# yu45020/Text_Segmentation_Image_Inpainting

Hardware: NVIDIA H100
Metric: PartialConv UNet 512x512 images/sec (fwd+bwd) (higher is better)
Workload: dtype bf16

## Files before the change

### text_segmentation_image_inpainting_b200/csrc/conv_tc.cu

```cuda
#include <cuda.h>
#include <stdlib.h>
#include <string.h>

#include <algorithm>

#include "pcb_common.cuh"
#include "pcb_ptx.cuh"
#include "pcb_tc_epi.cuh"

namespace {

__device__ __forceinline__ float warp_transpose_sum(float (&v)[32], int lane) {
#pragma unroll
    for (int off = 16, n = 32; off >= 1; off >>= 1, n >>= 1) {
        const bool upper = (lane & off) != 0;
#pragma unroll
        for (int i = 0; i < 16; ++i) {
            if (i < (n >> 1)) {
                const float send = upper ? v[i] : v[i + (n >> 1)];
                const float keep = upper ? v[i + (n >> 1)] : v[i];
                v[i] = keep + __shfl_xor_sync(0xffffffffu, send, off);
            }
        }
    }
// ... 621 lines not shown
                            const uint8_t *mk = P.parts[p].mask + static_cast<long long>(img) * (P.h >> mup) * (P.w >> mup);
                            for (int tr = 0; tr < P.kh; ++tr) {
                                const int y = oy - P.pad_h + tr * P.dil;
                                if (y < 0 || y >= P.h) continue;
#pragma unroll
                                for (int r = 0; r < FR; ++r) {
                                    const int row = t + TMA_FIX_THREADS * r, x = ox - P.pad_w + row;
                                    if (row < BLOCK_M + hx && x >= 0 && x < P.w && __ldg(mk + (y >> mup) * (P.w >> mup) + (x >> mup)) == 0)
                                        b[r] |= 1u << (p * 8 + tr);
                                }
                            }
                        }
                    };
                    uint32_t nb_bits[FR];
                    load_bits(tile0, nb_bits);
                    for (int tile = tile0; tile < num_tiles && !dead; tile += tstep) {
                        uint32_t cb_bits[FR];
#pragma unroll
                        for (int r = 0; r < FR; ++r) cb_bits[r] = nb_bits[r];
                        load_bits(tile + tstep, nb_bits);
                        if (MODE == 1 && !tile_active((tile % n_tiles) * BLOCK_N)) continue;
                        for (int tr = 0; tr < P.kh && !dead; ++tr) {
#pragma unroll
                            for (int p = 0; p < TC_MAX_PARTS; ++p) {
                                if (p >= np) break;
                                bool hole[FR], mine = false;
#pragma unroll
                                for (int r = 0; r < FR; ++r) { hole[r] = (cb_bits[r] >> (p * 8 + tr)) & 1u; mine = mine || hole[r]; }
                                const bool any_hole = __any_sync(0xffffffffu, mine);
                                const int nb = ((MODE == 0) ? P.parts[p].kext : P.dc_kext) / BLOCK_K;
                                for (int cb = 0; cb < nb; ++cb) {
                                    if (!ptx::mbar_wait(bar_full + 8 * s, ph, P.abort_flag, 122)) { dead = true; break; }
                                    if (any_hole) {
#pragma unroll
                                        for (int r = 0; r < FR; ++r)
                                            if (hole[r]) zero_row(t + TMA_FIX_THREADS * r);
                                        ptx::fence_proxy_async_smem();
                                    }
                                    __syncwarp();
                                    if (lane == 0) ptx::mbar_arrive(bar_fixed + 8 * s);
                                    if (++s == S) { s = 0; ph ^= 1; }
                                }
                                if (dead) break;
                            }
                        }
                    }
                }
            }
        }
    }

}


constexpr int SP_MAX_ITEMS = 40;
struct SpItem { int dx, dy, wk; };
struct SpTable {
    int n_items;
    SpItem it[SP_MAX_ITEMS];
};

template <int BLOCK_N>
__global__ void __maxnreg__(TMA_REGS)
pconv_tc_sp_kernel(const __grid_constant__ TcParams P, const __grid_constant__ SpTable TB, const __grid_constant__ CUtensorMap tmap_w,
                   const __grid_constant__ CUtensorMap tmap_a) {
    constexpr uint32_t B_BYTES = BLOCK_N * 128;
    constexpr uint32_t STAGE = A_STAGE_BYTES + B_BYTES;
    extern __shared__ uint8_t smem_raw[];
    const uint32_t smem_base = align1024(ptx::smem_u32(smem_raw));
    const int S = P.stages;
    const uint32_t sBar = smem_base + S * STAGE;
    const uint32_t bar_full = sBar, bar_empty = sBar + 16 * MAX_RING;
    const uint32_t acc_full = sBar + 24 * MAX_RING, acc_empty = acc_full + 8;
    const uint32_t s_acc = sBar + TMA_BAR_BYTES + EPI_STAT_SMEM_BYTES;
    bf16 *acc_stage = reinterpret_cast<bf16 *>(smem_raw + (s_acc - ptx::smem_u32(smem_raw)));

    const int warp = __shfl_sync(0xffffffffu, threadIdx.x >> 5, 0), lane = threadIdx.x & 31;
    const int n_tiles = P.ncols / BLOCK_N;
    const int m_tiles = (P.m_total + BLOCK_M - 1) / BLOCK_M;
    const int num_tiles = m_tiles * n_tiles;
    const int tile0 = static_cast<int>(blockIdx.x), tstep = static_cast<int>(gridDim.x);
    const int plane = P.w * P.h;
    const int nbk = P.dc_kext / BLOCK_K;
    const int klast = min(4, (P.dc_c8 - (nbk - 1) * BLOCK_K + 15) >> 4);

    if (threadIdx.x == 0) {
        for (int s = 0; s < MAX_RING; ++s) { ptx::mbar_init(bar_full + 8 * s, 1); ptx::mbar_init(bar_empty + 8 * s, 2); }
        ptx::mbar_init(acc_full, MMA_WARPS); ptx::mbar_init(acc_empty, EPI_WARPS);
        ptx::fence_mbar_init();
    }
    if (warp == 8 && lane == 0) { ptx::prefetch_tmap(&tmap_w); ptx::prefetch_tmap(&tmap_a); }
    __syncthreads();

    if (warp < MMA_WARPS) {
        ptx::setmaxnreg_inc<TMA_CONSUMER_REGS>();
        const int e = warp, g = warp >> 2;
        const bool leader = (threadIdx.x & 127) == 0;
        const uint64_t desc_a0 = ptx::make_smem_desc(smem_base + g * 64 * 128, 16, 1024);
        const uint64_t desc_b0 = ptx::make_smem_desc(smem_base + A_STAGE_BYTES, 16, 1024);
        const uint32_t stage16 = STAGE >> 4;
        int s = 0;
        uint32_t ph = 0, aph = 1;
        bool dead = false;
        for (int tile = tile0; tile < num_tiles && !dead; tile += tstep) {
            float acc[BLOCK_N / 2];
            zero_acc(acc);
// ... 824 lines not shown
bool even_upsampled_parts(const pcb_conv *c) {
    for (int p = 0; p < c->nparts; ++p)
        if (c->parts[p].x_up && ((c->h | c->w) & 1)) return false;
    return true;
}

bool tma_fwd_ok(const pcb_conv *c, int *bw, int *bh, int *bn) {
    if (is_rowpack(c) || !tile_box(c->wo, c->ho, bw, bh, bn)) return false;
    if (c->stride > 2 || *bw * c->stride > 256 || *bh * c->stride > 256) return false;
    return even_upsampled_parts(c);
}

bool tma_dgrad_s2_ok(const pcb_conv *c, int *bw, int *bh, int *bn) {
    if (c->stride != 2 || c->dil != 1 || c->kh < 2 || c->kw < 2 || ((c->h | c->w) & 1) || c->ho != c->h / 2 || c->wo != c->w / 2) return false;
    return tile_box(c->w / 2, c->h / 2, bw, bh, bn);
}

int class_kw(const pcb_conv *c, int px) { return (c->kw - ((px + c->pad_w) & 1) + 1) / 2; }

bool tma_wgrad_ok(const pcb_conv *c, int *bw, int *bh, int *bn) {
    return !is_rowpack(c) && c->stride <= 2 && kblock_box(c->wo, c->ho, bw, bh, bn) && even_upsampled_parts(c);
}

size_t up_bytes(const pcb_conv *c, int p) {
    return (static_cast<size_t>(c->n) * c->h * c->w * rup(c->parts[p].c, 8) * 2 + 255) / 256 * 256;
}
size_t tapmask_bytes(const pcb_conv *c) {
    return (static_cast<size_t>(c->nparts) * c->n * c->ho * c->wo * sizeof(uint64_t) + 255) / 256 * 256;
}

size_t tma_fixed_smem(int block_n) {
    return 1024 + TMA_BAR_BYTES + EPI_STAT_SMEM_BYTES + bf16_stage_bytes(block_n);
}

template <int BLOCK_N, int MODE, bool HALO>
int launch_tma_n(TcParams &P, const CUtensorMap &tw, const CUtensorMap &ta0, const CUtensorMap &ta1, cudaStream_t st) {
    const int nb = HALO ? P.kw : 1;
    const size_t a_room = (static_cast<size_t>(BLOCK_M + (HALO ? (P.kw - 1) * P.dil : 0)) * 128 + 1023) / 1024 * 1024;
    const size_t stage = a_room + static_cast<size_t>(nb) * BLOCK_N * 128;
    const size_t fixed = tma_fixed_smem(BLOCK_N);
    P.stages = static_cast<int>(std::min<size_t>(MAX_RING, (MAX_SMEM - fixed) / stage));
    PCB_CHECK(P.stages >= 2, "TMA-fed conv: stage of %zu bytes does not fit twice", stage);
    const size_t smem = fixed + P.stages * stage;
    auto kern = pconv_tc_tma_kernel<BLOCK_N, MODE, HALO>;
    PCB_SMEM_OPT_IN(kern, MAX_SMEM);
    const int m_tiles = (P.m_total + BLOCK_M - 1) / BLOCK_M;
    const int num_tiles = m_tiles * (P.ncols / BLOCK_N);
    const int grid = std::min(num_tiles, pcb_num_sms());
    kern<<<grid, TMA_THREADS, smem, st>>>(P, tw, ta0, ta1);
    PCB_LAUNCH_CHECK();
    return 0;
}

template <int MODE>
int launch_tma(TcParams &P, const CUtensorMap &tw, const CUtensorMap &ta0, const CUtensorMap &ta1, int bn, bool halo, cudaStream_t st) {
    PCB_CHECK(!(halo && bn == 256), "TMA-fed conv: no 256-wide row-halo tiles");
    if (halo) {
        if (bn == 128) return launch_tma_n<128, MODE, true>(P, tw, ta0, ta1, st);
        if (bn == 64) return launch_tma_n<64, MODE, true>(P, tw, ta0, ta1, st);
        return launch_tma_n<32, MODE, true>(P, tw, ta0, ta1, st);
    }
    if (bn == 256) return launch_tma_n<256, MODE, false>(P, tw, ta0, ta1, st);
    if (bn == 128) return launch_tma_n<128, MODE, false>(P, tw, ta0, ta1, st);
    if (bn == 64) return launch_tma_n<64, MODE, false>(P, tw, ta0, ta1, st);
    return launch_tma_n<32, MODE, false>(P, tw, ta0, ta1, st);
}

bool halo_stages_fit(int kw, int dil, int block_n) {
    const size_t stage = (static_cast<size_t>(128 + (kw - 1) * dil) * 128 + 1023) / 1024 * 1024 + static_cast<size_t>(kw) * block_n * 128;
    return 3 * stage + acc_stage_bytes(block_n) <= RING_BUDGET;
}

bool halo_ok(int kw, int dil, int bw, int bh, int bn, int block_n) {
    return bw == 128 && bh == 1 && bn == 1 && kw >= 2 && 128 + (kw - 1) * dil <= 256 && halo_stages_fit(kw, dil, block_n);
}

int pick_bn(int cols, long long m_total, bool fwd, int sms) {
    const long long m_tiles = (m_total + BLOCK_M - 1) / BLOCK_M;
    if (cols <= 32) return 32;
    auto waves = [&](int b) { return (m_tiles * (cols / b) + sms - 1) / sms; };
    if (cols % 256 == 0 && 2 * waves(256) <= waves(128) && (!fwd || waves(256) == 1)) return 256;
    int bn = (cols % 128 == 0) ? 128 : 64;
    while (bn > 32 && cols % (bn / 2) == 0 && m_tiles * (cols / bn) < sms / 2) bn /= 2;
    return bn;
}

template <int MODE>
int launch_tc(TcParams &P, const CUtensorMap &tm, int bn, cudaStream_t st) {
    return (bn == 128) ? launch_persistent<128, MODE>(P, tm, st) : launch_persistent<64, MODE>(P, tm, st);
}

struct ClassStreams { cudaStream_t aux[3]; cudaEvent_t ev_fork, ev_join[3]; bool ready; };
int class_streams(ClassStreams **out) {
    static thread_local ClassStreams cs_all[PCB_MAX_DEVICES] = {};
    ClassStreams &CS = cs_all[pcb_cur_device()];
    if (!CS.ready) {
        for (int i = 0; i < 3; ++i) {
            PCB_CUDA(cudaStreamCreateWithFlags(&CS.aux[i], cudaStreamNonBlocking));
            PCB_CUDA(cudaEventCreateWithFlags(&CS.ev_join[i], cudaEventDisableTiming));
        }
        PCB_CUDA(cudaEventCreateWithFlags(&CS.ev_fork, cudaEventDisableTiming));
        CS.ready = true;
    }
    *out = &CS;
    return 0;
}

struct SpAxis { int e0[2], ne[2], tapbits[2][4]; bool ok; };

// ... 108 lines not shown
    const int num_tiles = ((P.m_total + BLOCK_M - 1) / BLOCK_M) * (P.ncols / BLOCK_N);
    const int grid = std::min(num_tiles, pcb_num_sms());
    kern<<<grid, TMA_THREADS, smem, st>>>(P, TB, tw, ta);
    PCB_LAUNCH_CHECK();
    return 0;
}

int sp_dgrad_up(const pcb_conv *c, const SpPlan &S, const Layout &L, const void *dc, int dc_cstride, const bf16 *w_sp_dg, void *dx_u, int dx_cstride,
                int *flag, cudaStream_t st) {
    const int hs = c->h / 2, ws = c->w / 2;
    const long long m_src = static_cast<long long>(c->n) * hs * ws;
    TcParams P;
    base_params(P, c, L);
    P.h = hs; P.w = ws; P.m_total = static_cast<int>(m_src);
    P.sub = 1; P.py = 0; P.px = 0; P.fh = hs; P.fw = ws;
    P.nparts = 1;
    memset(P.parts, 0, sizeof(P.parts));
    TcPart &pt = P.parts[0];
    pt.c = c->parts[S.pu].c; pt.c8 = S.c8_u; pt.kext = S.kext_u; pt.koff = 0; pt.mask = c->parts[S.pu].mask; pt.mup = 0;
    pt.dx = static_cast<bf16 *>(dx_u); pt.dx_cstride = dx_cstride;
    PCB_CHECK(dx_cstride % 8 == 0 && dx_cstride >= S.c8_u && (reinterpret_cast<uintptr_t>(dx_u) & 15) == 0, "sub-pixel dgrad: dx must be 16-byte aligned with a channel stride that is a multiple of 8");
    P.dc = static_cast<const bf16 *>(dc); P.dc_cstride = dc_cstride; P.dc_c8 = rup(c->cout, 8); P.dc_kext = L.cout64;
    P.abort_flag = flag;
    P.ncols = S.kext_u;
    P.box_w = S.bw; P.box_h = S.bh; P.box_n = S.bn;
    const int bn = S.block_n;
    SpTable TB;
    memset(&TB, 0, sizeof(TB));
    int ni = 0;
    for (int cls = 0; cls < 4; ++cls) {
        const int py = cls >> 1, px = cls & 1;
        const int ney = S.ay.ne[py], nex = S.ax.ne[px];
        for (int e = 0; e < ney; ++e)
            for (int f = 0; f < nex; ++f) {
                SpItem &it = TB.it[ni++];
                it.dx = px - 2 * (S.ax.e0[px] + f); it.dy = py - 2 * (S.ay.e0[py] + e);
                it.wk = (S.eoff[cls] + e * nex + f) * L.cout64;
            }
    }
    TB.n_items = ni;
    CUtensorMap ta, tw;
    if (int rc = make_tmap_nhwc(&ta, dc, P.dc_c8, c->wo, c->ho, c->n, dc_cstride, S.bw, S.bh, S.bn, 2)) return rc;
    if (int rc = make_tmap_2d(&tw, w_sp_dg, rup(S.kext_u, 128), S.kd_sp, S.kd_sp, bn)) return rc;
    return (bn == 64) ? launch_sp_n<64>(P, TB, tw, ta, st) : launch_sp_n<32>(P, TB, tw, ta, st);
}

enum TcRoute { ROUTE_NONE, ROUTE_STEM, ROUTE_K2R, ROUTE_SMALLCO, ROUTE_TMA, ROUTE_TMA_S2, ROUTE_GATHER };

struct DirPlan {
    TcRoute route;
    int box_w, box_h, box_n;
    int bn;
    bool halo;
};

struct TcPlan {
    bool ok;
    Layout L;
    long long m_out, m_in;
    size_t fwd_elems, dg_elems;
    size_t extra_fwd_off, extra_dg_off;
    size_t sp_off;
    size_t workspace;
    size_t up_off[TC_MAX_PARTS];
    DirPlan fwd, dg, wg;
    bool fwd_tapmask, wg_tapmask;
    StemPlan stem;
    K2rPlan k2r;
    SpPlan sp;
    bool cls_halo[4];
    bool cls_fork;
    bool fuses_epilogue;
    bool dg_fuses_relu;
    bool dg_at_source;
};

TcPlan tc_plan(const pcb_conv *c) {
    TcPlan T;
    memset(&T, 0, sizeof(T));
    T.sp.pu = T.sp.ps = -1;
    if (!common_ok(c)) return T;
    T.ok = true;
    const int sms = pcb_num_sms();
    T.L = layout_of(c);
    const Layout &L = T.L;
    T.m_out = static_cast<long long>(c->n) * c->ho * c->wo;
    T.m_in = static_cast<long long>(c->n) * c->h * c->w;
    bool any_mask = false;
    for (int p = 0; p < c->nparts; ++p) any_mask = any_mask || (c->parts[p].mask != nullptr);
    const bool smallco = !L.rowpack && pcb_smallco_eligible(c);
    if (L.rowpack) T.stem = pcb_stem_plan(c);
    if (smallco) T.k2r = pcb_k2r_plan(c);
    const bool stem = T.stem.ok, k2r = T.k2r.ok;
    if (!L.rowpack && !smallco) T.sp = sp_plan(c, L, sms);

    T.fwd_elems = static_cast<size_t>(L.rows_f) * L.kf;
    T.sp_off = static_cast<size_t>(rup(L.ktap, 128)) * L.kd;
    T.dg_elems = L.rowpack ? 0 : T.sp_off;
    if (T.sp.ok) T.dg_elems += static_cast<size_t>(T.sp.sp_dg_elems);
    T.extra_fwd_off = (T.fwd_elems + 63) / 64 * 64;
    T.extra_dg_off = (T.sp_off + 63) / 64 * 64;
    if (k2r) {
        T.fwd_elems = T.extra_fwd_off + T.k2r.fwd_extra;
        T.dg_elems = T.extra_dg_off + T.k2r.dg_extra;
    }
    if (stem) T.fwd_elems = T.extra_fwd_off + T.stem.fwd_extra;

    int bw, bh, bn;
    const bool fwd_tma = tma_fwd_ok(c, &bw, &bh, &bn);
    DirPlan &F = T.fwd;
    if (stem) F.route = ROUTE_STEM;
    else if (k2r) F.route = ROUTE_K2R;
    else if (smallco) F.route = ROUTE_SMALLCO;
    else if (fwd_tma) {
        F.route = ROUTE_TMA;
        F.box_w = bw; F.box_h = bh; F.box_n = bn;
        F.bn = pick_bn(c->cout <= 32 ? 32 : L.rows_f, T.m_out, true, sms);
        F.halo = c->stride == 1 && c->kh <= 8 && halo_ok(c->kw, c->dil, bw, bh, bn, F.bn);
        T.fwd_tapmask = any_mask && !F.halo;
    } else {
        F.route = ROUTE_GATHER;
        F.bn = L.bn_f;
        T.fwd_tapmask = true;
    }

    DirPlan &D = T.dg;
    if (k2r) D.route = ROUTE_K2R;
    else if (smallco) D.route = ROUTE_SMALLCO;
    else if (L.rowpack) D.route = ROUTE_NONE;
    else if (c->stride == 1 && tile_box(c->w, c->h, &bw, &bh, &bn)) {
        D.route = ROUTE_TMA;
        D.box_w = bw; D.box_h = bh; D.box_n = bn;
        D.bn = pick_bn(L.ktap, T.m_in, false, sms);
        D.halo = c->kh <= 8 && halo_ok(c->kw, c->dil, bw, bh, bn, D.bn);
    } else if (tma_dgrad_s2_ok(c, &bw, &bh, &bn)) {
        D.route = ROUTE_TMA_S2;
        D.box_w = bw; D.box_h = bh; D.box_n = bn;
        const long long m_class = static_cast<long long>(c->n) * (c->h / 2) * (c->w / 2);
        D.bn = pick_bn(L.ktap, m_class, false, sms);
        for (int cls = 0; cls < 4; ++cls) T.cls_halo[cls] = halo_ok(class_kw(c, cls & 1), 1, bw, bh, bn, D.bn);
        T.cls_fork = ((m_class + BLOCK_M - 1) / BLOCK_M) * (L.ktap / D.bn) < sms;
    } else {
        D.route = ROUTE_GATHER;
        D.bn = (L.ktap % 128 == 0) ? 128 : 64;
    }

    const bool wg_tma = tma_wgrad_ok(c, &bw, &bh, &bn);
    DirPlan &W = T.wg;
    if (stem) W.route = ROUTE_STEM;
    else if (k2r) W.route = ROUTE_K2R;
    else if (smallco) W.route = ROUTE_SMALLCO;
    else if (wg_tma) {
        W.route = ROUTE_TMA;
        W.box_w = bw; W.box_h = bh; W.box_n = bn;
        W.halo = c->stride == 1 && c->kw == 3 && bw == 64 && bh == 1 && bn == 1 && 64 + (c->kw - 1) * c->dil <= 256;
        W.bn = (c->cout > 64 && T.m_out >= 128 * 64) ? 128 : 64;
        T.wg_tapmask = any_mask;
    } else {
        W.route = ROUTE_GATHER;
        T.wg_tapmask = true;
    }

    if (k2r) T.workspace = T.k2r.workspace;
    else if (stem) T.workspace = std::max(T.stem.workspace, tapmask_bytes(c));
    else {
        T.workspace = tapmask_bytes(c);
        if (fwd_tma || wg_tma)
            for (int p = 0; p < c->nparts; ++p)
                if (c->parts[p].x_up) { T.up_off[p] = T.workspace; T.workspace += up_bytes(c, p); }
    }

    T.fuses_epilogue = !smallco;
    T.dg_fuses_relu = c->nparts == 1 && !T.sp.ok && D.route == ROUTE_TMA;
    T.dg_at_source = smallco ? k2r : T.sp.ok;
    return T;
}

int a_operand_maps(const pcb_conv *c, const TcPlan &T, void *workspace, int bx, int by, int bn, CUtensorMap (&ta)[TC_MAX_PARTS],
                   int *use_fix, cudaStream_t st) {
    memset(ta, 0, sizeof(ta));
    for (int p = 0; p < c->nparts; ++p) {
        const pcb_part &pt = c->parts[p];
        const void *src = pt.x;
        long long cs = pt.x_cstride;
        const int c8 = rup(pt.c, 8);
        if (pt.x_up) {
            bf16 *up = reinterpret_cast<bf16 *>(static_cast<uint8_t *>(workspace) + T.up_off[p]);
// ... 65 lines not shown
    if (T.fwd.route == ROUTE_STEM) return pcb_stem_weight_prepare(c, T.stem, w_master, wf + T.extra_fwd_off, zero_padding, st);
    if (T.fwd.route == ROUTE_K2R) {
        PCB_CHECK(w_dgrad != nullptr, "kernel-to-row weights need the dgrad operand buffer");
        return pcb_k2r_weight_prepare(c, T.k2r, w_master, wf + T.extra_fwd_off, wd + T.extra_dg_off, zero_padding, st);
    }
    if (T.sp.ok) {
        PCB_CHECK(w_dgrad != nullptr, "sub-pixel weights need the dgrad operand buffer");
        return sp_weight_prepare(c, T.sp, L, w_master, wd + T.sp_off, st);
    }
    return 0;
}

int pcb_tc_forward_mask_pass(const pcb_conv *c, uint64_t *tapmask, cudaStream_t st) {
    const TcPlan T = tc_plan(c);
    PCB_CHECK(T.m_out < (1ll << 31), "problem too large");
    return T.fwd_tapmask ? launch_tapmask(c, tapmask, st) : 0;
}

bool pcb_tc_fuses_epilogue(const pcb_conv *c) { return tc_plan(c).fuses_epilogue; }

int pcb_tc_forward_ws(const pcb_conv *c, const void *w_fwd, const float *bias, void *y, int y_cstride, const float *msum,
                      uint64_t *tapmask, bool mask_pass_done, double *bn_sums, const pcb_ep *ep, cudaStream_t st) {
    int *flag = abort_flag_ptr();
    PCB_CHECK(flag != nullptr, "cudaMalloc(abort flag) failed");
    const TcPlan T = tc_plan(c);
    const Layout &L = T.L;
    const DirPlan &F = T.fwd;
    PCB_CHECK(T.m_out < (1ll << 31), "problem too large");
    PCB_CHECK(y_cstride % 8 == 0 && y_cstride >= c->cout, "tensor-core forward: y channel stride must be a multiple of 8 and >= cout");
    PCB_CHECK(bn_sums == nullptr || T.fuses_epilogue, "fused BatchNorm statistics requested from a kernel that does not produce them");
    PCB_CHECK(ep == nullptr || T.fuses_epilogue, "fused BatchNorm + activation requested from a kernel that does not apply it");
    if (!mask_pass_done && T.fwd_tapmask)
        if (int rc = launch_tapmask(c, tapmask, st)) return rc;
    const bf16 *wf = static_cast<const bf16 *>(w_fwd);
    if (F.route == ROUTE_STEM) return pcb_stem_forward(c, T.stem, wf + T.extra_fwd_off, bias, y, y_cstride, msum, tapmask, bn_sums, ep, st);
    if (F.route == ROUTE_K2R) return pcb_k2r_forward(c, T.k2r, smallco_layout(L), w_fwd, wf + T.extra_fwd_off, bias, y, y_cstride, msum, tapmask, st);
    if (F.route == ROUTE_SMALLCO) return pcb_smallco_forward(c, smallco_layout(L), w_fwd, bias, y, y_cstride, msum, st);
    TcParams P;
    base_params(P, c, L);
    P.m_total = static_cast<int>(T.m_out);
    fill_parts(c, L, P.parts, tapmask, T.m_out);
    P.bias = bias; P.msum = msum; P.y = static_cast<bf16 *>(y); P.y_cstride = y_cstride; P.abort_flag = flag;
    P.bn_sums = bn_sums; P.bn_c = c->cout;
    set_ep(P, ep);
    P.ncols = L.rows_f;
    CUtensorMap tm;
    if (int rc = make_tmap_2d(&tm, w_fwd, L.rows_f, L.kf, L.kf, F.bn)) return rc;
    if (F.route == ROUTE_TMA) {
        P.box_w = F.box_w; P.box_h = F.box_h; P.box_n = F.box_n;
        CUtensorMap ta[TC_MAX_PARTS];
        if (int rc = a_operand_maps(c, T, tapmask, F.box_w + (F.halo ? (c->kw - 1) * c->dil : 0), F.box_h, F.box_n, ta, &P.use_fix, st)) return rc;
        P.ncols = (c->cout <= 32) ? 32 : L.rows_f;
        P.wk_base = 0; P.wk_col = L.ktap; P.wk_row = c->kw * L.ktap;
        return launch_tma<0>(P, tm, ta[0], ta[1], F.bn, F.halo, st);
    }
    return launch_tc<0>(P, tm, F.bn, st);
}

bool pcb_tc_dgrad_fuses_relu(const pcb_conv *c) { return tc_plan(c).dg_fuses_relu; }

int pcb_tc_dgrad(const pcb_conv *c, const void *dc, int dc_cstride, const void *w_dgrad, void *const *dx, const int *dx_cstride,
                 cudaStream_t st, const void *relu_x, int relu_cstride) {
    const TcPlan T = tc_plan(c);
    const Layout &L = T.L;
    const DirPlan &D = T.dg;
    PCB_CHECK(D.route != ROUTE_NONE, "data gradient of a row-packed (cin <= 8) tensor-core layer: set force_generic and pass KRSC weights");
    PCB_CHECK(w_dgrad != nullptr && (reinterpret_cast<uintptr_t>(dc) & 15) == 0, "pcb_pconv_backward_data: w_dgrad required / dc misaligned");
    PCB_CHECK(relu_x == nullptr || (T.dg_fuses_relu && relu_cstride % 8 == 0 && relu_cstride >= rup(c->cin, 8) &&
                                    (reinterpret_cast<uintptr_t>(relu_x) & 15) == 0),
              "tensor-core dgrad: the ReLU backward is fused only on the TMA-fed stride-1 kernel (16-byte aligned input, channel stride %% 8 == 0)");
    int *flag = abort_flag_ptr();
    PCB_CHECK(flag != nullptr, "cudaMalloc(abort flag) failed");
    PCB_CHECK(T.m_in < (1ll << 31), "problem too large");
    PCB_CHECK(dc_cstride % 8 == 0 && dc_cstride >= rup(c->cout, 8), "tensor-core dgrad: dc channel stride must be a multiple of 8");
    const bf16 *wd = static_cast<const bf16 *>(w_dgrad);
    if (D.route == ROUTE_K2R) return pcb_k2r_dgrad(c, T.k2r, smallco_layout(L), dc, dc_cstride, w_dgrad, wd + T.extra_dg_off, dx, dx_cstride, st);
    if (D.route == ROUTE_SMALLCO) return pcb_smallco_dgrad(c, smallco_layout(L), dc, dc_cstride, w_dgrad, dx, dx_cstride, st);
    const SpPlan &SPL = T.sp;
    void *dx_local[TC_MAX_PARTS] = {nullptr, nullptr};
    for (int p = 0; p < c->nparts && p < TC_MAX_PARTS; ++p) dx_local[p] = dx[p];
    if (SPL.ok) {
        if (dx[SPL.pu] != nullptr)
            if (int rc = sp_dgrad_up(c, SPL, L, dc, dc_cstride, wd + T.sp_off, dx[SPL.pu], dx_cstride[SPL.pu], flag, st)) return rc;
        dx_local[SPL.pu] = nullptr;
        if (SPL.ps < 0 || dx[SPL.ps] == nullptr) return 0;
    }
    dx = dx_local;
    TcParams P;
    base_params(P, c, L);
    P.m_total = static_cast<int>(T.m_in);
    fill_parts(c, L, P.parts, nullptr, 0);
    for (int p = 0; p < c->nparts; ++p) {
        P.parts[p].dx = static_cast<bf16 *>(dx[p]);
        P.parts[p].dx_cstride = dx_cstride[p];
        PCB_CHECK(!dx[p] || (dx_cstride[p] % 8 == 0 && dx_cstride[p] >= P.parts[p].c8 && (reinterpret_cast<uintptr_t>(dx[p]) & 15) == 0),
                  "tensor-core dgrad: dx[%d] must be 16-byte aligned with a channel stride that is a multiple of 8", p);
    }
    P.dc = static_cast<const bf16 *>(dc); P.dc_cstride = dc_cstride; P.dc_c8 = rup(c->cout, 8); P.dc_kext = L.cout64;
    P.relu_x = static_cast<const bf16 *>(relu_x); P.relu_cstride = relu_cstride;
    P.abort_flag = flag;
    P.ncols = L.ktap;
    CUtensorMap tm;
    if (int rc = make_tmap_2d(&tm, w_dgrad, rup(L.ktap, 128), L.kd, L.kd, D.bn)) return rc;
    if (D.route == ROUTE_TMA) {
        P.box_w = D.box_w; P.box_h = D.box_h; P.box_n = D.box_n;
        P.wk_base = 0; P.wk_col = L.cout64; P.wk_row = c->kw * L.cout64;
        CUtensorMap ta;
        if (int rc = make_tmap_nhwc(&ta, dc, P.dc_c8, c->wo, c->ho, c->n, dc_cstride, D.box_w + (D.halo ? (c->kw - 1) * c->dil : 0), D.box_h, D.box_n, 1)) return rc;
        return launch_tma<1>(P, tm, ta, ta, D.bn, D.halo, st);
    }
    if (D.route == ROUTE_TMA_S2) {
        const int hh = c->h / 2, hw = c->w / 2;
        P.box_w = D.box_w; P.box_h = D.box_h; P.box_n = D.box_n;
        const bool fork = T.cls_fork;
        ClassStreams *CS = nullptr;
        if (fork) {
            if (int rc = class_streams(&CS)) return rc;
            PCB_CUDA(cudaEventRecord(CS->ev_fork, st));
        }
        for (int cls = 0; cls < 4; ++cls) {
            TcParams Q = P;
            const int py = cls >> 1, px = cls & 1;
            const int tr0 = (py + c->pad_h) & 1, tc0 = (px + c->pad_w) & 1;
            Q.kh = (c->kh - tr0 + 1) / 2; Q.kw = class_kw(c, px);
            Q.pad_h = (py + c->pad_h - tr0) / 2; Q.pad_w = (px + c->pad_w - tc0) / 2;
            Q.h = hh; Q.w = hw; Q.stride = 1; Q.dil = 1;
            Q.m_total = static_cast<int>(static_cast<long long>(c->n) * hh * hw);
            Q.sub = 2; Q.py = py; Q.px = px; Q.fh = c->h; Q.fw = c->w;
            Q.wk_base = (tr0 * c->kw + tc0) * L.cout64; Q.wk_row = 2 * c->kw * L.cout64; Q.wk_col = 2 * L.cout64;
            const bool halo = T.cls_halo[cls];
            CUtensorMap ta;
            if (int rc = make_tmap_nhwc(&ta, dc, P.dc_c8, c->wo, c->ho, c->n, dc_cstride, Q.box_w + (halo ? Q.kw - 1 : 0), Q.box_h, Q.box_n, 1)) return rc;
            cudaStream_t cs = (fork && cls > 0) ? CS->aux[cls - 1] : st;
            if (fork && cls > 0) PCB_CUDA(cudaStreamWaitEvent(cs, CS->ev_fork, 0));
            if (int rc = launch_tma<1>(Q, tm, ta, ta, D.bn, halo, cs)) return rc;
            if (fork && cls > 0) {
                PCB_CUDA(cudaEventRecord(CS->ev_join[cls - 1], cs));
                PCB_CUDA(cudaStreamWaitEvent(st, CS->ev_join[cls - 1], 0));
            }
        }
        return 0;
    }
    return launch_tc<1>(P, tm, D.bn, st);
}


template <int BLOCK_N, int T, bool HALO>
int launch_wgrad_tma(WgParams &P, const CUtensorMap &tdc, const CUtensorMap &ta0, const CUtensorMap &ta1, cudaStream_t st) {
    const int rows_a = 64 + (HALO ? (P.kw - 1) * P.dil : 0);
    PCB_CHECK(rows_a <= (HALO ? 3 : 1) * WGRAD_FIX_THREADS, "TMA-fed wgrad: %d-row A blocks exceed the fixer warps", rows_a);
    const size_t a_blk = (static_cast<size_t>(rows_a) * 128 + 1023) / 1024 * 1024;
    const size_t stage = (HALO ? 1 : T) * 2 * a_blk + static_cast<size_t>(BLOCK_N) * 128;
    P.stages = static_cast<int>(std::min<size_t>(MAX_RING, RING_BUDGET / stage));
    PCB_CHECK(P.stages >= 2, "TMA-fed wgrad: stage of %zu bytes does not fit twice", stage);
    const size_t smem = 1024 + P.stages * stage + 24 * MAX_RING;
    auto kern = pconv_tc_wgrad_tma_kernel<BLOCK_N, T, HALO>;
    PCB_SMEM_OPT_IN(kern, MAX_SMEM);
    P.tap_groups = HALO ? P.kh : (P.kh * P.kw + T - 1) / T;
    P.ci_tiles = (P.ktap + 127) / 128;
    const int co_tiles = (P.cout + BLOCK_N - 1) / BLOCK_N;
    const int base_ctas = co_tiles * P.tap_groups * P.ci_tiles;
    const int total_kb = (P.m_total + 63) / 64;
// ... 78 lines not shown
```

### text_segmentation_image_inpainting_b200/csrc/pcb_tc_epi.cuh

```cuda
#pragma once
#include <cuda.h>

#include "pcb_common.cuh"
#include "pcb_ptx.cuh"

namespace {

constexpr int BLOCK_M = 128;
constexpr int BLOCK_K = 64;
constexpr int A_STAGE_BYTES = BLOCK_M * 128;
constexpr int NUM_PRODUCER_THREADS = 128;
constexpr int TC_MAX_PARTS = 2;
constexpr int MMA_WARPS = 8;
constexpr int MMA_THREADS = MMA_WARPS * 32;
constexpr int acc_pitch(int block_n) { return block_n + 4; }
constexpr int acc_stage_bytes(int block_n) { return BLOCK_M * acc_pitch(block_n) * 4; }

inline int rup(int v, int m) { return (v + m - 1) / m * m; }

struct TcPart {
    const bf16 *x;
    const uint64_t *tapmask;
    const uint8_t *mask;
    bf16 *dx;
// ... 173 lines not shown
                ob[j] = __floats2bfloat162_rn(f.x * scale, f.y * scale);
            }
        }
        if (MODE == 1 && P.relu_x != nullptr && nstore > 0) {
            const uint4 *xr = reinterpret_cast<const uint4 *>(P.relu_x + er.mo * P.relu_cstride + xlocal);
#pragma unroll 1
            for (int j = 0; j < 4; ++j) {
                if (j * 8 >= nstore) break;
                const uint4 xv = xr[j];
                const __nv_bfloat162 *xb = reinterpret_cast<const __nv_bfloat162 *>(&xv);
                __nv_bfloat162 *ob = reinterpret_cast<__nv_bfloat162 *>(&o[j]);
#pragma unroll
                for (int k = 0; k < 4; ++k) {
                    const float2 xf = __bfloat1622float2(xb[k]);
                    const __nv_bfloat162 z = __float2bfloat162_rn(0.f);
                    ob[k] = __halves2bfloat162(xf.x <= 0.f ? z.x : ob[k].x, xf.y <= 0.f ? z.y : ob[k].y);
                }
            }
        }
        if (nstore > 0) {
            uint4 *dst = reinterpret_cast<uint4 *>(orow);
#pragma unroll
            for (int j = 0; j < 4; ++j)
                if (j * 8 < nstore) dst[j] = o[j];
        }
        if (stats) {
            const float live = er.rvalid ? 1.f : 0.f;
            const __nv_bfloat162 *ob = reinterpret_cast<const __nv_bfloat162 *>(srow + c0);
            float cs = 0.f, cq = 0.f;
#pragma unroll 1
            for (int h = 0; h < 2; ++h) {
                float v[16];
#pragma unroll
                for (int j = 0; j < 8; ++j) {
                    const float2 f = __bfloat1622float2(ob[8 * h + j]);
                    v[2 * j] = f.x * live; v[2 * j + 1] = f.y * live;
                }
                const float s = warp_transpose_sum16(v, lane);
#pragma unroll
                for (int j = 0; j < 8; ++j) {
                    const float2 f = __bfloat1622float2(ob[8 * h + j]);
                    const float a = f.x * live, b = f.y * live;
                    v[2 * j] = a * a; v[2 * j + 1] = b * b;
                }
                const float q = warp_transpose_sum16(v, lane);
                if ((lane >> 4) == h) { cs = s; cq = q; }
            }
            s_stat[c0 + lane] += cs;
            s_stat[EPI_STAT_SQ + c0 + lane] += cq;
        }
    }
}

template <int BLOCK_N, int MODE, typename TileFn>
__device__ __forceinline__ void tma_epilogue_warps(const TcParams &P, int tile0, int tstep, int num_tiles, TileFn tile_origin,
                                                   const bf16 *stage, uint32_t acc_full, uint32_t acc_empty, float *s_stat,
                                                   int &stat_n0, int w, int lane, int code) {
    const int row = w * 32 + lane;
    if (s_stat) {
        for (int i = lane; i < EPI_STAT_SLICE; i += 32) s_stat[i] = 0.f;
        __syncwarp();
    }
    uint32_t ph = 0;
    for (int tile = tile0; tile < num_tiles; tile += tstep) {
        int m0, n0;
        tile_origin(tile, m0, n0);
        if (n0 < 0) continue;
        if (s_stat && n0 != stat_n0) {
            if (stat_n0 >= 0) tc_stats_flush<BLOCK_N>(P, s_stat, lane, stat_n0, 0, BLOCK_N, EPI_STAT_SQ);
            stat_n0 = n0;
        }
        const EpiRow er = tc_epi_row<MODE>(P, m0 + row, false);
        if (!__all_sync(0xffffffffu, ptx::mbar_wait(acc_full, ph, P.abort_flag, code))) { stat_n0 = -1; return; }
        ph ^= 1;
        tc_epilogue_bf16<BLOCK_N, MODE>(P, er, stage + row * bf16_pitch(BLOCK_N), lane, n0, s_stat);
        __syncwarp();
        if (lane == 0) ptx::mbar_arrive(acc_empty);
    }
}

struct ConsRows {
    float inv[2];
    bool hole[2];
};
template <int MODE>
__device__ __forceinline__ ConsRows cons_rows(const TcParams &P, int m0, int e, int lane) {
    ConsRows cr;
#pragma unroll
    for (int h = 0; h < 2; ++h) {
        cr.inv[h] = 0.f; cr.hole[h] = false;
        if (MODE == 0) {
            const EpiRow er = tc_epi_row<0>(P, m0 + 64 * (e >> 2) + 16 * (e & 3) + (lane >> 2) + 8 * h);
            cr.inv[h] = er.inv; cr.hole[h] = er.hole;
        }
    }
    return cr;
}

template <int BLOCK_N, int MODE>
__device__ __forceinline__ void stage_acc_bf16(const TcParams &P, const float (&acc)[BLOCK_N / 2], bf16 *stage, int e, int lane, int n0,
                                               const ConsRows &cr) {
    constexpr int PITCH = bf16_pitch(BLOCK_N);
    const int r0 = 64 * (e >> 2) + 16 * (e & 3) + (lane >> 2), c0 = 2 * (lane & 3);
    const bool has_bias = (MODE == 0) && (P.bias != nullptr);
    const bool ep = (MODE == 0) && (P.ep_on != 0);
    const bool ep_aff = ep && (P.ep_scale != nullptr);
#pragma unroll
    for (int j = 0; j < BLOCK_N / 8; ++j) {
        const int col = n0 + 8 * j + c0;
        float b0 = 0.f, b1 = 0.f, s0 = 1.f, s1 = 1.f, t0 = 0.f, t1 = 0.f;
        if (MODE == 0) {
            const bool in0 = col < P.cout, in1 = col + 1 < P.cout;
            if (has_bias) { if (in0) b0 = __ldg(P.bias + col); if (in1) b1 = __ldg(P.bias + col + 1); }
            if (ep_aff) {
                if (in0) { s0 = __ldg(P.ep_scale + col); t0 = __ldg(P.ep_shift + col); }
                if (in1) { s1 = __ldg(P.ep_scale + col + 1); t1 = __ldg(P.ep_shift + col + 1); }
            }
        }
#pragma unroll
        for (int h = 0; h < 2; ++h) {
            float a = acc[4 * j + 2 * h], b = acc[4 * j + 2 * h + 1];
            if (MODE == 0) {
                a = cr.hole[h] ? 0.f : fmaf(a, cr.inv[h], b0);
                b = cr.hole[h] ? 0.f : fmaf(b, cr.inv[h], b1);
                if (ep) {
                    a = apply_act(fmaf(a, s0, t0), P.ep_act, P.ep_slope);
                    b = apply_act(fmaf(b, s1, t1), P.ep_act, P.ep_slope);
                }
                if (col >= P.cout) a = 0.f;
                if (col + 1 >= P.cout) b = 0.f;
            }
            *reinterpret_cast<__nv_bfloat162 *>(stage + (r0 + 8 * h) * PITCH + 8 * j + c0) = __floats2bfloat162_rn(a, b);
        }
    }
}

template <int BLOCK_N, int MODE>
__device__ __forceinline__ bool tma_stage_tile(const TcParams &P, const float (&acc)[BLOCK_N / 2], bf16 *stage, uint32_t acc_full,
                                               uint32_t acc_empty, uint32_t &ph, int e, int lane, int n0, const ConsRows &cr, int code) {
    if (!__all_sync(0xffffffffu, ptx::mbar_wait(acc_empty, ph, P.abort_flag, code))) return false;
    ph ^= 1;
    stage_acc_bf16<BLOCK_N, MODE>(P, acc, stage, e, lane, n0, cr);
    __syncwarp();
    if (lane == 0) ptx::mbar_arrive(acc_full);
    return true;
}

}
```

Measured before the change: 1163.

## Add pair-tile row-halo TMA conv kernel sharing weight stages across two M sub-tiles

Adds a kernel variant in which each CTA processes two adjacent 128-row row-halo sub-tiles. The two consumer warpgroups share each weight (B) stage, and A and W get separate ring buffers sized independently. The change targets weight-load traffic and barrier overhead per unit of MMA work on large stride-1 forward and dgrad convolutions. It costs more shared memory per stage, more accumulator registers (two sets per warp), and fewer tiles to spread across SMs. The planner enables it only when the tile count is at least twice the SM count.

```diff
diff --git a/text_segmentation_image_inpainting_b200/csrc/conv_tc.cu b/text_segmentation_image_inpainting_b200/csrc/conv_tc.cu
--- a/text_segmentation_image_inpainting_b200/csrc/conv_tc.cu
+++ b/text_segmentation_image_inpainting_b200/csrc/conv_tc.cu
@@ -697,6 +697,279 @@
 
 }
 
+constexpr size_t PAIR_BAR_BYTES = 40 * MAX_RING + 16;
+
+template <int BLOCK_N, int MODE, bool HALO, int PAIRS>
+__global__ void __maxnreg__(TMA_REGS)
+pconv_tc_tma_kernel(const __grid_constant__ TcParams P, const __grid_constant__ CUtensorMap tmap_w,
+                    const __grid_constant__ CUtensorMap tmap_a0, const __grid_constant__ CUtensorMap tmap_a1) {
+    static_assert(HALO && PAIRS == 2 && (BLOCK_N == 64 || BLOCK_N == 128), "pair tiles: two row-halo sub-tiles, N = 64 or 128");
+    constexpr int PM = PAIRS * BLOCK_M;
+    constexpr uint32_t B_BYTES = BLOCK_N * 128;
+    extern __shared__ uint8_t smem_raw[];
+    const uint32_t smem_base = align1024(ptx::smem_u32(smem_raw));
+    const int SA = P.ring_a, SW = P.ring_b;
+    const int hx = (P.kw - 1) * P.dil;
+    const int rows_sub = BLOCK_M + hx;
+    const uint32_t A_BYTES = static_cast<uint32_t>(rows_sub) * 128u;
+    const uint32_t A_ROOM = (A_BYTES + 1023u) & ~1023u;
+    const uint32_t ASTAGE = PAIRS * A_ROOM;
+    const uint32_t sW = smem_base + SA * ASTAGE;
+    const uint32_t sBar = sW + SW * B_BYTES;
+    const uint32_t a_full = sBar, a_fixed = sBar + 8 * MAX_RING, a_empty = sBar + 16 * MAX_RING;
+    const uint32_t w_full = sBar + 24 * MAX_RING, w_empty = sBar + 32 * MAX_RING;
+    const uint32_t acc_full = sBar + 40 * MAX_RING, acc_empty = acc_full + 8;
+    const uint32_t s_stat_addr = sBar + PAIR_BAR_BYTES;
+    const uint32_t s_acc = s_stat_addr + EPI_STAT_SMEM_BYTES;
+    uint8_t *smem_gen = smem_raw + (smem_base - ptx::smem_u32(smem_raw));
+
+    const int warp = __shfl_sync(0xffffffffu, threadIdx.x >> 5, 0), lane = threadIdx.x & 31;
+    const int np = (MODE == 0) ? P.nparts : 1;
+    const int n_tiles = P.ncols / BLOCK_N;
+    const int num_tiles = (P.m_total / PM) * n_tiles;
+    const int tile0 = static_cast<int>(blockIdx.x), tstep = static_cast<int>(gridDim.x);
+    const bool fix = (MODE == 0) && P.use_fix;
+
+    auto tile_active = [&](int n0) -> bool {
+        if (MODE == 0) return true;
+        for (int p = 0; p < P.nparts; ++p)
+            if (P.parts[p].dx && n0 < P.parts[p].koff + P.parts[p].kext && n0 + BLOCK_N > P.parts[p].koff) return true;
+        return false;
+    };
+
+    if (threadIdx.x == 0) {
+        for (int s = 0; s < MAX_RING; ++s) {
+            ptx::mbar_init(a_full + 8 * s, 1); ptx::mbar_init(a_fixed + 8 * s, TMA_FIX_THREADS / 32); ptx::mbar_init(a_empty + 8 * s, 2);
+            ptx::mbar_init(w_full + 8 * s, 1); ptx::mbar_init(w_empty + 8 * s, 2);
+        }
+        ptx::mbar_init(acc_full, MMA_WARPS); ptx::mbar_init(acc_empty, EPI_WARPS);
+        ptx::fence_mbar_init();
+    }
+    if (warp == 8 && lane == 0) { ptx::prefetch_tmap(&tmap_w); ptx::prefetch_tmap(&tmap_a0); if (np > 1) ptx::prefetch_tmap(&tmap_a1); }
+    __syncthreads();
+
+    bf16 *acc_stage = reinterpret_cast<bf16 *>(smem_gen + (s_acc - smem_base));
+    if (warp < MMA_WARPS) {
+        ptx::setmaxnreg_inc<TMA_CONSUMER_REGS>();
+        const int g = warp >> 2, we = warp & 3;
+        const bool leader = (threadIdx.x & 127) == 0;
+        const uint32_t ready = fix ? a_fixed : a_full;
+        const uint64_t desc_a0 = ptx::make_smem_desc(smem_base + g * A_ROOM, 16, 1024);
+        const uint64_t desc_b0 = ptx::make_smem_desc(sW, 16, 1024);
+        const uint32_t astage16 = ASTAGE >> 4, b16 = B_BYTES >> 4, half16 = (64 * 128) >> 4;
+        const int shift0 = (MODE == 1) ? hx * 8 : 0;
+        const int dshift = (MODE == 1) ? -P.dil * 8 : P.dil * 8;
+        int nb0, nb1 = 0, kl0, kl1 = 4;
+        {
+            const int kext = (MODE == 0) ? P.parts[0].kext : P.dc_kext, c8 = (MODE == 0) ? P.parts[0].c8 : P.dc_c8;
+            nb0 = kext / BLOCK_K; kl0 = min(4, (c8 - (nb0 - 1) * BLOCK_K + 15) >> 4);
+            if (MODE == 0 && np > 1) { nb1 = P.parts[1].kext / BLOCK_K; kl1 = min(4, (P.parts[1].c8 - (nb1 - 1) * BLOCK_K + 15) >> 4); }
+        }
+        int sa = 0, sw = 0;
+        uint32_t pha = 0, phw = 0, aph = 1;
+        bool dead = false;
+        for (int tile = tile0; tile < num_tiles && !dead; tile += tstep) {
+            const int n0 = (tile % n_tiles) * BLOCK_N;
+            if (!tile_active(n0)) continue;
+            const int m0 = (tile / n_tiles) * PM + g * BLOCK_M;
+            const ConsRows cr0 = cons_rows<MODE>(P, m0, we, lane), cr1 = cons_rows<MODE>(P, m0, we + 4, lane);
+            float acc0[BLOCK_N / 2], acc1[BLOCK_N / 2];
+            zero_acc(acc0);
+            zero_acc(acc1);
+            int held_a = -1, held_w = -1;
+            for (int r = 0; r < P.kh && !dead; ++r) {
+#pragma unroll
+                for (int p = 0; p < TC_MAX_PARTS; ++p) {
+                    const int nbp = (p == 0) ? nb0 : nb1, klast = (p == 0) ? kl0 : kl1;
+                    for (int cb = 0; cb < nbp && !dead; ++cb) {
+                        if (!__all_sync(0xffffffffu, ptx::mbar_wait(ready + 8 * sa, pha, P.abort_flag, 144))) { dead = true; break; }
+                        uint64_t da = desc_a0 + static_cast<uint64_t>(sa * astage16 + shift0);
+                        const int ksteps = (cb + 1 < nbp) ? 4 : klast;
+                        for (int tc = 0; tc < P.kw; ++tc, da += dshift) {
+                            if (!__all_sync(0xffffffffu, ptx::mbar_wait(w_full + 8 * sw, phw, P.abort_flag, 145))) { dead = true; break; }
+                            const uint64_t db = desc_b0 + static_cast<uint64_t>(sw * b16);
+                            ptx::wgmma_fence();
+                            if (ksteps == 4) {
+#pragma unroll
+                                for (int k = 0; k < 4; ++k) {
+                                    ptx::wgmma_bf16<BLOCK_N, 0, 0>(acc0, da + 2 * k, db + 2 * k);
+                                    ptx::wgmma_bf16<BLOCK_N, 0, 0>(acc1, da + half16 + 2 * k, db + 2 * k);
+                                }
+                            } else {
+                                for (int k = 0; k < ksteps; ++k) {
+                                    ptx::wgmma_bf16<BLOCK_N, 0, 0>(acc0, da + 2 * k, db + 2 * k);
+                                    ptx::wgmma_bf16<BLOCK_N, 0, 0>(acc1, da + half16 + 2 * k, db + 2 * k);
+                                }
+                            }
+                            ptx::wgmma_commit();
+                            ptx::wgmma_wait<1>();
+                            if (leader) {
+                                if (held_w >= 0) ptx::mbar_arrive(w_empty + 8 * held_w);
+                                if (held_a >= 0) ptx::mbar_arrive(a_empty + 8 * held_a);
+                            }
+                            held_a = -1;
+                            held_w = sw;
+                            if (++sw == SW) { sw = 0; phw ^= 1; }
+                        }
+                        held_a = sa;
+                        if (++sa == SA) { sa = 0; pha ^= 1; }
+                    }
+                    if (dead) break;
+                }
+            }
+            ptx::wgmma_wait<0>();
+            ptx::wgmma_fence_regs(acc0);
+            ptx::wgmma_fence_regs(acc1);
+            if (leader) {
+                if (held_w >= 0) ptx::mbar_arrive(w_empty + 8 * held_w);
+                if (held_a >= 0) ptx::mbar_arrive(a_empty + 8 * held_a);
+            }
+            if (dead) break;
+            if (!__all_sync(0xffffffffu, ptx::mbar_wait(acc_empty, aph, P.abort_flag, 146))) break;
+            aph ^= 1;
+            stage_acc_bf16_sets<BLOCK_N, MODE, true>(P, acc0, acc1, acc_stage + g * BLOCK_M * bf16_pitch(BLOCK_N), we, lane, n0, cr0, cr1);
+            __syncwarp();
+            if (lane == 0) ptx::mbar_arrive(acc_full);
+        }
+    } else {
+        ptx::setmaxnreg_dec<TMA_SUPPORT_REGS>();
+        if (warp >= EPI_WARP0) {
+            const int w = warp - EPI_WARP0;
+            float *s_stat = (MODE == 0 && P.bn_sums != nullptr)
+                                ? reinterpret_cast<float *>(smem_gen + (s_stat_addr - smem_base)) + w * EPI_STAT_SLICE : nullptr;
+            int stat_n0 = -1;
+            auto origin = [&](int tile, int &m0, int &n0) {
+                m0 = (tile / n_tiles) * PM; n0 = (tile % n_tiles) * BLOCK_N;
+                if (!tile_active(n0)) n0 = -1;
+            };
+            tma_epilogue_warps<BLOCK_N, MODE, PAIRS>(P, tile0, tstep, num_tiles, origin, acc_stage, acc_full, acc_empty, s_stat, stat_n0, w,
+                                                     lane, 147);
+            ptx::named_sync(1, EPI_WARPS * 32);
+            if (s_stat != nullptr && stat_n0 >= 0) tc_stats_final<BLOCK_N>(P, s_stat - w * EPI_STAT_SLICE, w, lane, stat_n0);
+        } else if (warp == 8) {
+            int sa = 0, sw = 0;
+            uint32_t pha = 1, phw = 1;
+            const int plane = (MODE == 0) ? P.ho * P.wo : P.h * P.w;
+            const int pwid = (MODE == 0) ? P.wo : P.w;
+            const int kext0 = (MODE == 0) ? P.parts[0].kext : P.dc_kext, kext1 = (MODE == 0 && np > 1) ? P.parts[1].kext : 0;
+            const int dstep = (MODE == 0) ? P.dil : -P.dil;
+            bool dead = false;
+            for (int tile = tile0; tile < num_tiles && !dead; tile += tstep) {
+                const int mp = (tile / n_tiles) * PM, n0 = (tile % n_tiles) * BLOCK_N;
+                if (!tile_active(n0)) continue;
+                int xs[PAIRS], ys[PAIRS], img[PAIRS];
+#pragma unroll
+                for (int j = 0; j < PAIRS; ++j) {
+                    const int m = mp + j * BLOCK_M;
+                    img[j] = m / plane;
+                    const int rem = m - img[j] * plane, oy = rem / pwid, ox = rem - oy * pwid;
+                    xs[j] = (MODE == 0) ? ox - P.pad_w : ox + P.pad_w - hx;
+                    ys[j] = (MODE == 0) ? oy - P.pad_h : oy + P.pad_h;
+                }
+                int krow = P.wk_base;
+                for (int tr = 0; tr < P.kh && !dead; ++tr, krow += P.wk_row) {
+                    int kidx = krow;
+#pragma unroll
+                    for (int p = 0; p < TC_MAX_PARTS; ++p) {
+                        const int kext = (p == 0) ? kext0 : kext1;
+                        const CUtensorMap *ma = (p == 0) ? &tmap_a0 : &tmap_a1;
+                        for (int c0 = 0; c0 < kext && !dead; c0 += BLOCK_K, kidx += BLOCK_K) {
+                            if (!__all_sync(0xffffffffu, ptx::mbar_wait(a_empty + 8 * sa, pha, P.abort_flag, 141))) { dead = true; break; }
+                            if (ptx::elect_one()) {
+                                const uint32_t full = a_full + 8 * sa, dst = smem_base + sa * ASTAGE;
+                                ptx::mbar_arrive_expect_tx(full, PAIRS * A_BYTES);
+#pragma unroll
+                                for (int j = 0; j < PAIRS; ++j) ptx::tma_load_4d(dst + j * A_ROOM, ma, c0, xs[j], ys[j] + tr * dstep, img[j], full);
+                            }
+                            __syncwarp();
+                            if (++sa == SA) { sa = 0; pha ^= 1; }
+                            for (int tc = 0; tc < P.kw; ++tc) {
+                                if (!__all_sync(0xffffffffu, ptx::mbar_wait(w_empty + 8 * sw, phw, P.abort_flag, 142))) { dead = true; break; }
+                                if (ptx::elect_one()) {
+                                    const uint32_t full = w_full + 8 * sw;
+                                    ptx::mbar_arrive_expect_tx(full, B_BYTES);
+                                    ptx::tma_load_2d(sW + sw * B_BYTES, &tmap_w, kidx + tc * P.wk_col, n0, full);
+                                }
+                                __syncwarp();
+                                if (++sw == SW) { sw = 0; phw ^= 1; }
+                            }
+                        }
+                        if (dead) break;
+                    }
+                }
+            }
+        } else if (fix) {
+            constexpr int FR = 3;
+            const int t = (warp - 9) * 32 + lane;
+            auto box_of = [&](int r) -> int { return t + TMA_FIX_THREADS * r >= rows_sub ? 1 : 0; };
+            auto row_of = [&](int r) -> int { return t + TMA_FIX_THREADS * r - box_of(r) * rows_sub; };
+            const int plane = P.ho * P.wo;
+            int sa = 0;
+            uint32_t pha = 0;
+            bool dead = false;
+            auto load_bits = [&](int tl) -> uint64_t {
+                uint64_t b = 0;
+                if (tl >= num_tiles) return b;
+                const int mp = (tl / n_tiles) * PM;
+#pragma unroll
+                for (int r = 0; r < FR; ++r) {
+                    if (t + TMA_FIX_THREADS * r >= PAIRS * rows_sub) continue;
+                    const int m = mp + box_of(r) * BLOCK_M;
+                    const int img = m / plane, rem = m - img * plane;
+                    const int oy = rem / P.wo, ox = rem - oy * P.wo;
+                    const int x = ox - P.pad_w + row_of(r);
+                    if (x < 0 || x >= P.w) continue;
+#pragma unroll
+                    for (int p = 0; p < TC_MAX_PARTS; ++p) {
+                        if (p >= P.nparts || P.parts[p].mask == nullptr) continue;
+                        const int mup = P.parts[p].mup;
+                        const uint8_t *mk = P.parts[p].mask + static_cast<long long>(img) * (P.h >> mup) * (P.w >> mup);
+                        for (int tr = 0; tr < P.kh; ++tr) {
+                            const int y = oy - P.pad_h + tr * P.dil;
+                            if (y >= 0 && y < P.h && __ldg(mk + (y >> mup) * (P.w >> mup) + (x >> mup)) == 0) b |= 1ull << (16 * r + 8 * p + tr);
+                        }
+                    }
+                }
+                return b;
+            };
+            uint64_t nb_bits = load_bits(tile0);
+            for (int tile = tile0; tile < num_tiles && !dead; tile += tstep) {
+                const uint64_t cb_bits = nb_bits;
+                nb_bits = load_bits(tile + tstep);
+                for (int tr = 0; tr < P.kh && !dead; ++tr) {
+#pragma unroll
+                    for (int p = 0; p < TC_MAX_PARTS; ++p) {
+                        if (p >= np) break;
+                        bool hole[FR], mine = false;
+#pragma unroll
+                        for (int r = 0; r < FR; ++r) { hole[r] = (cb_bits >> (16 * r + 8 * p + tr)) & 1ull; mine = mine || hole[r]; }
+                        const bool any_hole = __any_sync(0xffffffffu, mine);
+                        const int nb = P.parts[p].kext / BLOCK_K;
+                        for (int cb = 0; cb < nb; ++cb) {
+                            if (!ptx::mbar_wait(a_full + 8 * sa, pha, P.abort_flag, 143)) { dead = true; break; }
+                            if (any_hole) {
+#pragma unroll
+                                for (int r = 0; r < FR; ++r)
+                                    if (hole[r]) {
+                                        uint4 *row = reinterpret_cast<uint4 *>(smem_gen + sa * ASTAGE + box_of(r) * A_ROOM + row_of(r) * 128);
+                                        const uint4 z = make_uint4(0u, 0u, 0u, 0u);
+#pragma unroll
+                                        for (int k = 0; k < 8; ++k) row[k] = z;
+                                    }
+                                ptx::fence_proxy_async_smem();
+                            }
+                            __syncwarp();
+                            if (lane == 0) ptx::mbar_arrive(a_fixed + 8 * sa);
+                            if (++sa == SA) { sa = 0; pha ^= 1; }
+                        }
+                        if (dead) break;
+                    }
+                }
+            }
+        }
+    }
+}
+
 
 constexpr int SP_MAX_ITEMS = 40;
 struct SpItem { int dx, dy, wk; };
@@ -1627,9 +1900,53 @@
     return 0;
 }
 
+size_t pair_fixed_smem(int block_n) {
+    return 1024 + PAIR_BAR_BYTES + EPI_STAT_SMEM_BYTES + 2 * bf16_stage_bytes(block_n);
+}
+
+bool pair_stages(int kw, int dil, int block_n, int *sa, int *sw) {
+    const long long a_stage = 2 * ((static_cast<long long>(BLOCK_M + (kw - 1) * dil) * 128 + 1023) / 1024 * 1024);
+    const long long w_stage = static_cast<long long>(block_n) * 128;
+    const long long room = static_cast<long long>(MAX_SMEM) - static_cast<long long>(pair_fixed_smem(block_n));
+    const long long want_w = std::min(MAX_RING, 2 * kw + 2);
+    int a = 2;
+    while (a < MAX_RING && room - (a + 1) * a_stage >= want_w * w_stage) ++a;
+    const long long w = room >= a * a_stage ? std::min<long long>(MAX_RING, (room - a * a_stage) / w_stage) : 0;
+    *sa = a; *sw = static_cast<int>(w);
+    return w >= kw + 1;
+}
+
+bool pair_ok(int kh, int kw, int dil, int bw, int bh, int bn, int block_n, long long m_total, int ncols, int sms) {
+    int sa, sw;
+    return bw == 128 && bh == 1 && bn == 1 && kh <= 8 && kw >= 2 && (block_n == 64 || block_n == 128) &&
+           2 * (BLOCK_M + (kw - 1) * dil) <= 3 * TMA_FIX_THREADS && m_total % (2 * BLOCK_M) == 0 &&
+           (m_total / (2 * BLOCK_M)) * (ncols / block_n) >= 2ll * sms && pair_stages(kw, dil, block_n, &sa, &sw);
+}
+
+template <int BLOCK_N, int MODE>
+int launch_tma_pair_n(TcParams &P, const CUtensorMap &tw, const CUtensorMap &ta0, const CUtensorMap &ta1, cudaStream_t st) {
+    PCB_CHECK(pair_stages(P.kw, P.dil, BLOCK_N, &P.ring_a, &P.ring_b) && P.m_total % (2 * BLOCK_M) == 0,
+              "TMA-fed conv: pair-tile rings do not fit");
+    const size_t a_room = (static_cast<size_t>(BLOCK_M + (P.kw - 1) * P.dil) * 128 + 1023) / 1024 * 1024;
+    const size_t smem = pair_fixed_smem(BLOCK_N) + P.ring_a * 2 * a_room + static_cast<size_t>(P.ring_b) * BLOCK_N * 128;
+    auto kern = pconv_tc_tma_kernel<BLOCK_N, MODE, true, 2>;
+    PCB_SMEM_OPT_IN(kern, MAX_SMEM);
+    const int num_tiles = (P.m_total / (2 * BLOCK_M)) * (P.ncols / BLOCK_N);
+    const int grid = std::min(num_tiles, pcb_num_sms());
+    kern<<<grid, TMA_THREADS, smem, st>>>(P, tw, ta0, ta1);
+    PCB_LAUNCH_CHECK();
+    return 0;
+}
+
 template <int MODE>
-int launch_tma(TcParams &P, const CUtensorMap &tw, const CUtensorMap &ta0, const CUtensorMap &ta1, int bn, bool halo, cudaStream_t st) {
+int launch_tma(TcParams &P, const CUtensorMap &tw, const CUtensorMap &ta0, const CUtensorMap &ta1, int bn, bool halo, cudaStream_t st,
+               bool pairs = false) {
     PCB_CHECK(!(halo && bn == 256), "TMA-fed conv: no 256-wide row-halo tiles");
+    if (pairs) {
+        PCB_CHECK(halo && (bn == 128 || (MODE == 1 && bn == 64)), "TMA-fed conv: pair tiles are 128-wide (data gradient: also 64-wide) row-halo tiles");
+        if constexpr (MODE == 0) return launch_tma_pair_n<128, MODE>(P, tw, ta0, ta1, st);
+        else return (bn == 128) ? launch_tma_pair_n<128, MODE>(P, tw, ta0, ta1, st) : launch_tma_pair_n<64, MODE>(P, tw, ta0, ta1, st);
+    }
     if (halo) {
         if (bn == 128) return launch_tma_n<128, MODE, true>(P, tw, ta0, ta1, st);
         if (bn == 64) return launch_tma_n<64, MODE, true>(P, tw, ta0, ta1, st);
@@ -1844,6 +2161,7 @@
     int box_w, box_h, box_n;
     int bn;
     bool halo;
+    bool pairs;
 };
 
 struct TcPlan {
@@ -1907,8 +2225,10 @@
     else if (fwd_tma) {
         F.route = ROUTE_TMA;
         F.box_w = bw; F.box_h = bh; F.box_n = bn;
-        F.bn = pick_bn(c->cout <= 32 ? 32 : L.rows_f, T.m_out, true, sms);
-        F.halo = c->stride == 1 && c->kh <= 8 && halo_ok(c->kw, c->dil, bw, bh, bn, F.bn);
+        const int ncols = c->cout <= 32 ? 32 : L.rows_f;
+        F.bn = pick_bn(ncols, T.m_out, true, sms);
+        F.pairs = c->stride == 1 && F.bn == 128 && pair_ok(c->kh, c->kw, c->dil, bw, bh, bn, F.bn, T.m_out, ncols, sms);
+        F.halo = F.pairs || (c->stride == 1 && c->kh <= 8 && halo_ok(c->kw, c->dil, bw, bh, bn, F.bn));
         T.fwd_tapmask = any_mask && !F.halo;
     } else {
         F.route = ROUTE_GATHER;
@@ -1924,7 +2244,8 @@
         D.route = ROUTE_TMA;
         D.box_w = bw; D.box_h = bh; D.box_n = bn;
         D.bn = pick_bn(L.ktap, T.m_in, false, sms);
-        D.halo = c->kh <= 8 && halo_ok(c->kw, c->dil, bw, bh, bn, D.bn);
+        D.pairs = pair_ok(c->kh, c->kw, c->dil, bw, bh, bn, D.bn, T.m_in, L.ktap, sms);
+        D.halo = D.pairs || (c->kh <= 8 && halo_ok(c->kw, c->dil, bw, bh, bn, D.bn));
     } else if (tma_dgrad_s2_ok(c, &bw, &bh, &bn)) {
         D.route = ROUTE_TMA_S2;
         D.box_w = bw; D.box_h = bh; D.box_n = bn;
@@ -2096,7 +2417,7 @@
         if (int rc = a_operand_maps(c, T, tapmask, F.box_w + (F.halo ? (c->kw - 1) * c->dil : 0), F.box_h, F.box_n, ta, &P.use_fix, st)) return rc;
         P.ncols = (c->cout <= 32) ? 32 : L.rows_f;
         P.wk_base = 0; P.wk_col = L.ktap; P.wk_row = c->kw * L.ktap;
-        return launch_tma<0>(P, tm, ta[0], ta[1], F.bn, F.halo, st);
+        return launch_tma<0>(P, tm, ta[0], ta[1], F.bn, F.halo, st, F.pairs);
     }
     return launch_tc<0>(P, tm, F.bn, st);
 }
@@ -2151,7 +2472,7 @@
         P.wk_base = 0; P.wk_col = L.cout64; P.wk_row = c->kw * L.cout64;
         CUtensorMap ta;
         if (int rc = make_tmap_nhwc(&ta, dc, P.dc_c8, c->wo, c->ho, c->n, dc_cstride, D.box_w + (D.halo ? (c->kw - 1) * c->dil : 0), D.box_h, D.box_n, 1)) return rc;
-        return launch_tma<1>(P, tm, ta, ta, D.bn, D.halo, st);
+        return launch_tma<1>(P, tm, ta, ta, D.bn, D.halo, st, D.pairs);
     }
     if (D.route == ROUTE_TMA_S2) {
         const int hh = c->h / 2, hw = c->w / 2;
diff --git a/text_segmentation_image_inpainting_b200/csrc/pcb_tc_epi.cuh b/text_segmentation_image_inpainting_b200/csrc/pcb_tc_epi.cuh
--- a/text_segmentation_image_inpainting_b200/csrc/pcb_tc_epi.cuh
+++ b/text_segmentation_image_inpainting_b200/csrc/pcb_tc_epi.cuh
@@ -249,7 +249,7 @@
     }
 }
 
-template <int BLOCK_N, int MODE, typename TileFn>
+template <int BLOCK_N, int MODE, int SUB = 1, typename TileFn>
 __device__ __forceinline__ void tma_epilogue_warps(const TcParams &P, int tile0, int tstep, int num_tiles, TileFn tile_origin,
                                                    const bf16 *stage, uint32_t acc_full, uint32_t acc_empty, float *s_stat,
                                                    int &stat_n0, int w, int lane, int code) {
@@ -271,6 +271,9 @@
         if (!__all_sync(0xffffffffu, ptx::mbar_wait(acc_full, ph, P.abort_flag, code))) { stat_n0 = -1; return; }
         ph ^= 1;
         tc_epilogue_bf16<BLOCK_N, MODE>(P, er, stage + row * bf16_pitch(BLOCK_N), lane, n0, s_stat);
+        if (SUB == 2)
+            tc_epilogue_bf16<BLOCK_N, MODE>(P, tc_epi_row<MODE>(P, m0 + BLOCK_M + row, false), stage + (BLOCK_M + row) * bf16_pitch(BLOCK_N),
+                                            lane, n0, s_stat);
         __syncwarp();
         if (lane == 0) ptx::mbar_arrive(acc_empty);
     }
@@ -294,9 +297,9 @@
     return cr;
 }
 
-template <int BLOCK_N, int MODE>
-__device__ __forceinline__ void stage_acc_bf16(const TcParams &P, const float (&acc)[BLOCK_N / 2], bf16 *stage, int e, int lane, int n0,
-                                               const ConsRows &cr) {
+template <int BLOCK_N, int MODE, bool TWO>
+__device__ __forceinline__ void stage_acc_bf16_sets(const TcParams &P, const float (&acc0)[BLOCK_N / 2], const float (&acc1)[BLOCK_N / 2],
+                                                    bf16 *stage, int e, int lane, int n0, const ConsRows &cr0, const ConsRows &cr1) {
     constexpr int PITCH = bf16_pitch(BLOCK_N);
     const int r0 = 64 * (e >> 2) + 16 * (e & 3) + (lane >> 2), c0 = 2 * (lane & 3);
     const bool has_bias = (MODE == 0) && (P.bias != nullptr);
@@ -315,21 +318,32 @@
             }
         }
 #pragma unroll
-        for (int h = 0; h < 2; ++h) {
-            float a = acc[4 * j + 2 * h], b = acc[4 * j + 2 * h + 1];
-            if (MODE == 0) {
-                a = cr.hole[h] ? 0.f : fmaf(a, cr.inv[h], b0);
-                b = cr.hole[h] ? 0.f : fmaf(b, cr.inv[h], b1);
-                if (ep) {
-                    a = apply_act(fmaf(a, s0, t0), P.ep_act, P.ep_slope);
-                    b = apply_act(fmaf(b, s1, t1), P.ep_act, P.ep_slope);
-                }
-                if (col >= P.cout) a = 0.f;
-                if (col + 1 >= P.cout) b = 0.f;
-            }
-            *reinterpret_cast<__nv_bfloat162 *>(stage + (r0 + 8 * h) * PITCH + 8 * j + c0) = __floats2bfloat162_rn(a, b);
-        }
-    }
+        for (int set = 0; set < (TWO ? 2 : 1); ++set) {
+            const float (&acc)[BLOCK_N / 2] = set ? acc1 : acc0;
+            const ConsRows &cr = set ? cr1 : cr0;
+#pragma unroll
+            for (int h = 0; h < 2; ++h) {
+                float a = acc[4 * j + 2 * h], b = acc[4 * j + 2 * h + 1];
+                if (MODE == 0) {
+                    a = cr.hole[h] ? 0.f : fmaf(a, cr.inv[h], b0);
+                    b = cr.hole[h] ? 0.f : fmaf(b, cr.inv[h], b1);
+                    if (ep) {
+                        a = apply_act(fmaf(a, s0, t0), P.ep_act, P.ep_slope);
+                        b = apply_act(fmaf(b, s1, t1), P.ep_act, P.ep_slope);
+                    }
+                    if (col >= P.cout) a = 0.f;
+                    if (col + 1 >= P.cout) b = 0.f;
+                }
+                *reinterpret_cast<__nv_bfloat162 *>(stage + (r0 + 64 * set + 8 * h) * PITCH + 8 * j + c0) = __floats2bfloat162_rn(a, b);
+            }
+        }
+    }
+}
+
+template <int BLOCK_N, int MODE>
+__device__ __forceinline__ void stage_acc_bf16(const TcParams &P, const float (&acc)[BLOCK_N / 2], bf16 *stage, int e, int lane, int n0,
+                                               const ConsRows &cr) {
+    stage_acc_bf16_sets<BLOCK_N, MODE, false>(P, acc, acc, stage, e, lane, n0, cr, cr);
 }
 
 template <int BLOCK_N, int MODE>
```

Measured after the change: 1177 (median of 6 runs). 1.2% higher.
